# ZSHCRWY25/3DRVO-MARL-CollisionAvoidance

Measured on AMD Instinct MI355X. Metric: drone-steps/sec (env.step throughput), higher is better.
Workload: dtype f64; 1 GPU; BASELINE config 3 env.step: 64 drones x 4096 envs per GPU, nm=10, 0 buildings, map [50.0, 50.0, 10.0], fused step+auto-reset, f32 actions in HBM; envs_per_gpu=4096, drones=64, diag_build=False, cold_all=False, ablate=0, device_error_word=0

## Files before the change

### 3drvo-marl-collisionavoidance_amd/csrc/rvo3d_aux_kernels.hpp

```cpp
#pragma once

#include "rvo3d_step.hpp"

namespace rvo3d {

__global__ void reset_kernel(const Params P, const uint8_t* env_mask, const uint8_t* drone_mask) {
  const int g = blockIdx.x * blockDim.x + threadIdx.x;
  if (g >= P.E * P.N) return;
  if (env_mask && !env_mask[g / P.N]) return;
  if (drone_mask && !drone_mask[g]) return;
  double s[3];
  load_wp(P, g, 0, s);
  P.px()[g] = s[0]; P.py()[g] = s[1]; P.pz()[g] = s[2];
  P.vx()[g] = 0.0; P.vy()[g] = 0.0; P.vz()[g] = 0.0;
  P.wp_idx()[g] = 1; P.arrive()[g] = 0; P.dest()[g] = 0;
  P.real_len()[g] = 0.0; P.max_dev()[g] = 0.0; P.yaw()[g] = 0.0; P.pitch()[g] = 0.0;
  double c1[3];
  load_wp(P, g, 1, c1);
  RVO3D_STORE_CUR(P, g, c1);
  RVO3D_STORE_PREV(P, g, s);
  const bool plain = P.dev0()[g] == 0.0;
  P.dvk_a()[g] = plain ? P.dv0_a()[g] : kDvInvalid;
  P.dvk_b()[g] = P.dv0_b()[g];
}

__global__ void wpcache_kernel(const Params P) {
  const int g = blockIdx.x * blockDim.x + threadIdx.x;
  if (g >= P.E * P.N) return;
  const int np = P.n_points()[g];
  int i = P.wp_idx()[g];
  i = i < 1 ? 1 : (i > np - 1 ? np - 1 : i);
  double v[3];
  load_wp(P, g, i, v);
  RVO3D_STORE_CUR(P, g, v);
  load_wp(P, g, i - 1, v);
  RVO3D_STORE_PREV(P, g, v);
}

__global__ void dv0_kernel(const Params P) {
  const int g = blockIdx.x * blockDim.x + threadIdx.x;
  if (g >= P.E * P.N) return;
  double p[3], cur[3], dv[3];
  load_wp(P, g, 0, p);
  load_wp(P, g, 1, cur);
  des_vel(P, p, cur, dv);
  uint32_t a, b;
  dv_encode(dv, a, b);
  P.dv0_a()[g] = a; P.dv0_b()[g] = b;
  P.dev0()[g] = deviation(p, cur, p);
}

__global__ void des_vel_kernel(const Params P, double* out) {
  const int g = blockIdx.x * blockDim.x + threadIdx.x;
  if (g >= P.E * P.N) return;
  double p[3] = {P.px()[g], P.py()[g], P.pz()[g]}, cur[3], dv[3];
  RVO3D_LOAD_CUR(P, g, cur);
  des_vel(P, p, cur, dv);
  out[3 * (size_t)g] = dv[0]; out[3 * (size_t)g + 1] = dv[1]; out[3 * (size_t)g + 2] = dv[2];
}

struct RvoVelArgs { double vmax[3]; double acceler; };

__device__ __forceinline__ int arange_len(double lo, double hi) {
  const double n = __builtin_ceil((hi - lo) / 0.5);
  return n > 0 ? (int)n : 0;
}
__device__ __forceinline__ double arange_at(double lo, int k) {
  const double next = lo + 0.5;
  return k == 0 ? lo : (k == 1 ? next : lo + k * (next - lo));
}

__global__ void __launch_bounds__(512) rvo_vel_kernel(const Params P, const RvoVelArgs A, double* out) {
  extern __shared__ __attribute__((aligned(16))) unsigned char smem[];
  const int N = P.N, d = threadIdx.x, e = blockIdx.x;
  const int T = blockDim.x;
  double* const lx = reinterpret_cast<double*>(smem);
  const bool active = d < N;
  const int g = active ? e * N + d : e * N;
  Drone S;
  S.x = P.px()[g]; S.y = P.py()[g]; S.z = P.pz()[g];
  S.vx = P.vx()[g]; S.vy = P.vy()[g]; S.vz = P.vz()[g];
// ... 130 lines not shown
```

### 3drvo-marl-collisionavoidance_amd/csrc/rvo3d_capi.hip

```cpp
#include "../../include/rvo3d.h"
#include "rvo3d_device.hpp"

#include <atomic>
#include <cmath>
#include <cstdio>
#include <cstdlib>
#include <cstring>
#include <exception>
#include <new>
#include <string>
#include <vector>

using rvo3d::Params;

namespace {
thread_local std::string g_err;

int fail(int code, const std::string& msg) {
  g_err = msg;
  return code;
}
#define HIP_TRY(expr)                                                            \
  do {                                                                           \
    hipError_t _e = (expr);                                                      \
// ... 317 lines not shown
  *out = nullptr;
  if (cfg->num_envs < 1 || cfg->num_drones < 1 || cfg->num_drones > rvo3d::kMaxThreads)
    return fail(RVO3D_ERR_INVALID, "need num_envs >= 1 and 1 <= num_drones <= 512");
  if (cfg->max_points < 2 || cfg->num_buildings < 0 || cfg->neighbors_num < 0)
    return fail(RVO3D_ERR_INVALID, "need max_points >= 2, num_buildings >= 0, neighbors_num >= 0");
  if ((long long)cfg->num_envs * cfg->num_drones > (1ll << 30))
    return fail(RVO3D_ERR_INVALID, "num_envs * num_drones too large");
  if (cfg->action_decimals > 9) return fail(RVO3D_ERR_INVALID, "action_decimals must be <= 9");
  DeviceGuard dg;
  if (int rc0 = dg.enter(cfg->device)) return rc0;

  rvo3d_env* h = new (std::nothrow) rvo3d_env();
  if (!h) return fail(RVO3D_ERR_INVALID, "out of host memory");
  struct Owner {
    rvo3d_env* p;
    ~Owner() {
      if (!p) return;
      if (p->arena) (void)hipFree(p->arena);
      delete p;
    }
  } owner{h};
  h->cfg = *cfg;
  Params& P = h->P;
  rvo3d::Cold& C = h->cold;
  std::memset(&P, 0, sizeof P);
  std::memset(&C, 0, sizeof C);
  P.E = cfg->num_envs; P.N = cfg->num_drones; P.P = cfg->max_points;
  C.nb = cfg->num_buildings; P.nm = cfg->neighbors_num; P.env_train = cfg->env_train ? 1 : 0;
  P.W = 12 + 9 * P.nm;
#ifdef RVO3D_DIAG
  if (const char* ab = std::getenv("RVO3D_ABLATE")) P.ablate = std::atoi(ab);
#endif
  C.act_scale = cfg->action_decimals >= 0 ? std::pow(10.0, cfg->action_decimals) : 0.0;
  for (int k = 0; k < 3; ++k) C.map[k] = cfg->map_size[k];
  P.T10 = sq_threshold(10.0);
  C.T5 = sq_threshold(5.0);
  C.bgx = C.bgy = 0; C.bg_inv = 0.0;
  if (cfg->num_buildings > 0 && cfg->map_size[0] > 0 && cfg->map_size[1] > 0 &&
      std::isfinite(cfg->map_size[0]) && std::isfinite(cfg->map_size[1])) {
    const double cs = std::fmax(8.0, std::fmax(cfg->map_size[0], cfg->map_size[1]) / 64.0);
    C.bgx = (int)std::ceil(cfg->map_size[0] / cs); C.bgy = (int)std::ceil(cfg->map_size[1] / cs);
    if (C.bgx < 1) C.bgx = 1;
    if (C.bgy < 1) C.bgy = 1;
    C.bg_inv = 1.0 / cs;
  }
  C.T04 = sq_threshold(0.4);
  {
    double mx = std::fmax(C.map[0], std::fmax(C.map[1], C.map[2]));
    if (!(mx > 0)) mx = 1.0;
    for (int k = 0; k < 3; ++k) C.cen[k] = 0.5 * C.map[k];
    const double cmax = 0.75 * mx + 16.0;
    const double u = std::ldexp(1.0, -24);
    const double eD = u * (2.0 * cmax + 21.0);
    const double band = 2.0 * (2.0 * 1.7320508 * 10.5 * eD + 3.0 * eD * eD + 8.0 * u * 110.25);
    C.cmax = (float)cmax;
    P.band = std::nextafter((float)band, INFINITY);
    const float t10f = std::nextafter((float)(P.T10 + band), INFINITY);
    P.t10n = -std::nextafter(t10f, INFINITY);
    P.bandn = P.band + P.t10n;
    C.kdot = std::nextafter((float)(2.0 * (eD + 4.0 * u * 10.5) * 1.001), INFINITY);
    const double gap = 512.0 * band;
    const double cs = 4.0 * (1.7320508 * eD / std::sqrt(gap) + 8.0 * u);
    P.x1_gap = (float)gap;
    P.x1_k2 = (float)(1.0 - (4e-3 + 4.0 * cs));
    const double cs_out = cs > 1e-3 ? cs : 1e-3;
    P.x1_cs2 = (float)(cs_out * cs_out);
// ... 85 lines not shown
  RVO3D_API_BEGIN
  DeviceGuard dg;
  int rc = check(h, false, dg);
  if (rc) return rc;
  if (!waypoints || !n_points) return fail(RVO3D_ERR_INVALID, "waypoints / n_points are required");
  const Params& P = h->P;
  const rvo3d::Cold& C = h->cold;
  if (C.nb > 0 && !buildings) return fail(RVO3D_ERR_INVALID, "buildings required when num_buildings > 0");
  hipStream_t s = static_cast<hipStream_t>(stream);
  const size_t EN = (size_t)P.E * P.N;
  std::vector<double> wp((size_t)P.P * 3 * EN), rl(EN), rad(EN), pri(EN), p95(P.P);
  for (size_t g = 0; g < EN; ++g) {
    const int np = n_points[g];
    if (np < 2 || np > P.P) return fail(RVO3D_ERR_INVALID, "n_points entries must be in [2, max_points]");
    const double* src = waypoints + g * P.P * 3;
    double total = 0.0;
    for (int k = 0; k < P.P; ++k) {
      const int kk = k < np ? k : np - 1;
      for (int c = 0; c < 3; ++c) wp[((size_t)k * 3 + c) * EN + g] = src[kk * 3 + c];
      if (k + 1 < np) {
        const double dx = src[(k + 1) * 3] - src[k * 3], dy = src[(k + 1) * 3 + 1] - src[k * 3 + 1],
                     dz = src[(k + 1) * 3 + 2] - src[k * 3 + 2];
        total += std::sqrt(py_sq(dx) + py_sq(dy) + py_sq(dz));
      }
    }
    rl[g] = total;
    rad[g] = radius ? radius[g] : 0.2;
    pri[g] = priority ? priority[g] : 5.0;
  }
  {
    bool uni = true;
    for (size_t g = 1; g < EN && uni; ++g)
      uni = std::memcmp(&rad[g], &rad[0], 8) == 0 && std::memcmp(&pri[g], &pri[0], 8) == 0;
    h->P.uniform_rp = uni ? 1 : 0;
    h->P.r0 = rad[0];
    h->P.prio0 = pri[0];
  }
  for (int k = 0; k < P.P; ++k) p95[k] = std::pow(0.95, (double)k);
  HIP_TRY(hipMemcpy2DAsync((void*)P.wp(0, 0), (size_t)P.S * 8, wp.data(), EN * 8, EN * 8,
                           (size_t)P.P * 3, hipMemcpyHostToDevice, s));
  HIP_TRY(hipMemcpyAsync((void*)P.n_points(), n_points, EN * 4, hipMemcpyHostToDevice, s));
  HIP_TRY(hipMemcpyAsync((void*)P.route_len(), rl.data(), EN * 8, hipMemcpyHostToDevice, s));
  HIP_TRY(hipMemcpyAsync((void*)P.radius(), rad.data(), EN * 8, hipMemcpyHostToDevice, s));
  HIP_TRY(hipMemcpyAsync((void*)P.prio(), pri.data(), EN * 8, hipMemcpyHostToDevice, s));
  HIP_TRY(hipMemcpyAsync((void*)C.pow95, p95.data(), (size_t)P.P * 8, hipMemcpyHostToDevice, s));
  std::vector<uint16_t> grid;
  if (C.nb > 0) {
    HIP_TRY(hipMemcpyAsync((void*)C.bld, buildings, (size_t)C.nb * 32, hipMemcpyHostToDevice, s));
    if (C.bgx > 0) {
      const int K = rvo3d::kBgridK;
      const double cs = 1.0 / C.bg_inv;
      double rmax = 0.0;
      for (size_t g = 0; g < EN; ++g) {
        if (rad[g] != rad[g]) rmax = INFINITY;
        else if (rad[g] > rmax) rmax = rad[g];
      }
      grid.assign((size_t)C.bgx * C.bgy * (K + 1), 0);
      for (int ix = 0; ix < C.bgx; ++ix)
        for (int iy = 0; iy < C.bgy; ++iy) {
          uint16_t* cell = &grid[((size_t)ix * C.bgy + iy) * (K + 1)];
          const double x0 = ix == 0 ? -INFINITY : ix * cs, x1 = ix == C.bgx - 1 ? INFINITY : (ix + 1) * cs;
          const double y0 = iy == 0 ? -INFINITY : iy * cs, y1 = iy == C.bgy - 1 ? INFINITY : (iy + 1) * cs;
          int n = 0;
          bool overflow = false;
          for (int b = 0; b < C.nb && !overflow; ++b) {
            const double bx = buildings[4 * b], by = buildings[4 * b + 1];
            double reach = rmax + buildings[4 * b + 3];
            if (!(reach < 5.0)) reach = 5.0;
            reach += 1e-3;
// ... 552 lines not shown
```

### 3drvo-marl-collisionavoidance_amd/csrc/rvo3d_math.hpp

```cpp
#pragma once

#include "rvo3d_params.hpp"

namespace rvo3d {

__device__ __forceinline__ double sq(double x) { return x * x; }
__device__ __forceinline__ double dot3b(double ax, double ay, double az, double bx,
                                        double by, double bz) {
  return __builtin_fma(az, bz, __builtin_fma(ay, by, ax * bx));
}
__device__ __forceinline__ double norm3b(double x, double y, double z) {
  return __builtin_sqrt(dot3b(x, y, z, x, y, z));
}
__device__ __forceinline__ double norm2sq(double x, double y) { return __builtin_fma(y, y, x * x); }
__device__ __forceinline__ bool finite_d(double q) { return __builtin_fabs(q) < __builtin_inf(); }

__device__ __forceinline__ float round2_f32(double x) {
  const double k = __builtin_rint(x * 100.0);
  return __builtin_fabs(k) < 16777216.0 ? (float)(k * 0.01) : (float)(k / 100.0);
}
__device__ __forceinline__ double k_over_1000(double k) {
  const double q = k * 0.001;
  const double r = __builtin_fma(-q, 1000.0, k);
  const double c = q + r * 0.001;
  return finite_d(k) ? c : k;
}

constexpr uint32_t kDvInvalid = 0xffffffffu;
__device__ __forceinline__ void dv_encode(const double dv[3], uint32_t& a, uint32_t& b) {
  const double k0 = __builtin_rint(dv[0] * 1000.0), k1 = __builtin_rint(dv[1] * 1000.0),
               k2 = __builtin_rint(dv[2] * 1000.0);
  const bool ok = __builtin_fabs(k0) <= 1023.0 && __builtin_fabs(k1) <= 1023.0 &&
                  __builtin_fabs(k2) <= 1023.0 && k_over_1000(k0) == dv[0] &&
                  k_over_1000(k1) == dv[1] && k_over_1000(k2) == dv[2];
  const uint32_t nz = (uint32_t)(k0 == 0.0 && __builtin_signbit(dv[0])) |
                      ((uint32_t)(k1 == 0.0 && __builtin_signbit(dv[1])) << 1) |
                      ((uint32_t)(k2 == 0.0 && __builtin_signbit(dv[2])) << 2);
  a = ok ? ((uint32_t)((int)k0 + 1024) | ((uint32_t)((int)k1 + 1024) << 16)) : kDvInvalid;
  b = (uint32_t)((int)(ok ? k2 : 0.0) + 1024) | (nz << 16);
}
__device__ __forceinline__ bool dv_decode(uint32_t a, uint32_t b, double dv[3]) {
  if (a == kDvInvalid) return false;
  const int k0 = (int)(a & 0xffffu) - 1024, k1 = (int)(a >> 16) - 1024, k2 = (int)(b & 0xffffu) - 1024;
  dv[0] = (b & (1u << 16)) ? -0.0 : k_over_1000((double)k0);
  dv[1] = (b & (1u << 17)) ? -0.0 : k_over_1000((double)k1);
  dv[2] = (b & (1u << 18)) ? -0.0 : k_over_1000((double)k2);
  return true;
}

__device__ __forceinline__ double py_round2_c(double x) {
  double p = x * 100.0;
  double e = __builtin_fma(x, 100.0, -p);
  double c = __builtin_floor(p);
  double d = (p - (c + 0.5)) + e;
  if (d > 0.0) c += 1.0;
  else if (d == 0.0 && (((long long)c) & 1)) c += 1.0;
  return c;
}
__device__ __forceinline__ double clampd(double x, double lo, double hi) {
  return x < lo ? lo : (x > hi ? hi : x);
}
__device__ __forceinline__ double np_mod(double a, double b) {
  double m;
  if (b > 0.0 && a > -b && a < 2.0 * b) m = a >= b ? a - b : a;
  else m = fmod(a, b);
  if (m != 0.0) {
    if ((b < 0.0) != (m < 0.0)) m += b;
  } else {
    m = __builtin_copysign(0.0, b);
  }
  return m;
}

__device__ __forceinline__ void des_vel(const Params& P, const double p[3], const double cur[3],
                                        double out[3]) {
  const double dx = cur[0] - p[0], dy = cur[1] - p[1], dz = cur[2] - p[2];
  const double d2 = dot3b(dx, dy, dz, dx, dy, dz);
  if (d2 > P.cold().T04) {
    const double inv = 1000.0 / __builtin_sqrt(d2);
    const double ux = dx * inv, uy = dy * inv, uz = dz * inv;
    double kx = __builtin_rint(ux), ky = __builtin_rint(uy), kz = __builtin_rint(uz);
    const double m = __builtin_fmin(__builtin_fmin(0.5 - __builtin_fabs(ux - kx),
                                                   0.5 - __builtin_fabs(uy - ky)),
                                    0.5 - __builtin_fabs(uz - kz));
    if (!(m > 1e-7)) {
      const double az = atan2(dy, dx);
      const double el = atan2(dz, __builtin_sqrt(norm2sq(dx, dy)));
      double sa, ca, se, ce;
      sincos(az, &sa, &ca);
      sincos(el, &se, &ce);
      kx = __builtin_rint((1.0 * (ca * ce)) * 1000.0);
      ky = __builtin_rint((1.0 * (sa * ce)) * 1000.0);
      kz = __builtin_rint((1.0 * se) * 1000.0);
    }
    out[0] = k_over_1000(kx); out[1] = k_over_1000(ky); out[2] = k_over_1000(kz);
  } else {
    out[0] = out[1] = out[2] = 0.0;
  }
}

__device__ __forceinline__ double deviation(const double a[3], const double b[3],
                                            const double p[3]) {
  double dx = b[0] - a[0], dy = b[1] - a[1], dz = b[2] - a[2];
  double mag = __builtin_sqrt(sq(dx) + sq(dy) + sq(dz));
  if (mag == 0.0) return 0.0;
  double hx = dx / mag, hy = dy / mag, hz = dz / mag;
  double qx0 = p[0] - a[0], qy0 = p[1] - a[1], qz0 = p[2] - a[2];
  double t = qx0 * hx + qy0 * hy + qz0 * hz;
  double qx = a[0] + t * hx, qy = a[1] + t * hy, qz = a[2] + t * hz;
  return __builtin_sqrt(sq(p[0] - qx) + sq(p[1] - qy) + sq(p[2] - qz));
}

__device__ __forceinline__ bool arrived(const Params& P, const double p[3], const double d[3]) {
  const double x = p[0] - d[0], y = p[1] - d[1], z = p[2] - d[2];
  return dot3b(x, y, z, x, y, z) <= P.cold().T04;
}

__device__ __forceinline__ double vo_exp_time(double rx, double ry, double rz, double rvx,
                                              double rvy, double rvz, double ra, double rb) {
  double r = ra + rb;
  double ux = -rvx, uy = -rvy, uz = -rvz;
  double a = sq(ux) + sq(uy) + sq(uz);
  double b = 2 * rx * ux + 2 * ry * uy + 2 * rz * uz;
  double c = sq(rx) + sq(ry) + sq(rz) - sq(r);
  if (c <= 0) return 0.0;
  double temp = sq(b) - 4 * a * c;
  if (temp <= 0) return __builtin_inf();
  double s = __builtin_sqrt(temp);
  double t1 = (-b + s) / (2 * a);
  double t2 = (-b - s) / (2 * a);
  if (t1 < 0 && t2 < 0) return -1.0;
// ... 17 lines not shown
```

### 3drvo-marl-collisionavoidance_amd/csrc/rvo3d_params.hpp

```cpp
#pragma once

#include <hip/hip_runtime.h>
#include <stdint.h>

namespace rvo3d {

constexpr double kExpRadius = 0.2;
constexpr double kCtimeThreshold = 2.0;
constexpr double kDeg2Rad = 0.017453292519943295;
constexpr double kPi = 3.141592653589793;
constexpr int kMaxThreads = 512;
constexpr double kCosD = 0.999999995;
constexpr double kSinD = 1.0000000000e-4;

struct Cold {
  double map[3];
  double T5, T04;
  double cen[3];
  double act_scale;
  float cmax;
  float kdot;
  uint32_t zf_div;
  uint32_t zf_magic;
  uint32_t zf_q;
  int zf_iters;
  uint32_t zmask[128];
  int nb;
  const double* bld;
  const double* pow95;
  const uint16_t* bgrid;
  int bgx, bgy;
  double bg_inv;
};
constexpr int kBgridK = 15;
typedef const __attribute__((address_space(4))) Cold ColdC;

struct Params {
  int E, N, P, nm, env_train, epb, W;
  int action_f64;
  int dv_cached;
  int g_cached;
  int action_mode;
  float acceler;
#ifdef RVO3D_DIAG
  int ablate;
#endif
  int zf16;
  int uniform_rp;
  double r0, prio0;
  double T10;
  float t10n;
  float bandn;
  float band;
  int nw;
  float x1_gap;
  float x1_k2;
  float x1_cs2;
  double* f64;
  int32_t* i32;
  uint8_t* u8;
  uint32_t S;
  enum { F_PX, F_PY, F_PZ, F_VX, F_VY, F_VZ, F_YAW, F_PITCH, F_REAL_LEN, F_MAX_DEV, F_EXTRA_LEN,
         F_CUR, F_PREV = F_CUR + 3,
         F_ROUTE_LEN = F_PREV + 3, F_RADIUS, F_PRIO, F_DEV0, F_WP };
  __host__ __device__ double* f(int k) const { return f64 + (size_t)k * S; }
  __host__ __device__ double* px() const { return f(F_PX); }
  __host__ __device__ double* py() const { return f(F_PY); }
  __host__ __device__ double* pz() const { return f(F_PZ); }
  __host__ __device__ double* vx() const { return f(F_VX); }
  __host__ __device__ double* vy() const { return f(F_VY); }
  __host__ __device__ double* vz() const { return f(F_VZ); }
  __host__ __device__ double* yaw() const { return f(F_YAW); }
  __host__ __device__ double* pitch() const { return f(F_PITCH); }
  __host__ __device__ double* real_len() const { return f(F_REAL_LEN); }
  __host__ __device__ double* max_dev() const { return f(F_MAX_DEV); }
  __host__ __device__ double* extra_len() const { return f(F_EXTRA_LEN); }
  __host__ __device__ int32_t* wp_idx() const { return i32; }
  __host__ __device__ uint8_t* arrive() const { return u8; }
  __host__ __device__ uint8_t* dest() const { return u8 + S; }
  __host__ __device__ double* route_len() const { return f(F_ROUTE_LEN); }
  __host__ __device__ double* radius() const { return f(F_RADIUS); }
  __host__ __device__ double* prio() const { return f(F_PRIO); }
// ... 44 lines not shown
```

### 3drvo-marl-collisionavoidance_amd/csrc/rvo3d_step.hpp

```cpp
#pragma once

#include "rvo3d_pairs.hpp"

namespace rvo3d {

__device__ __forceinline__ bool building_test(const double* const bld, int b, const Drone& S,
                                              double T5) {
  const double bx = bld[4 * b], by = bld[4 * b + 1], bh = bld[4 * b + 2], br = bld[4 * b + 3];
  const double ex = S.x - bx, ey = S.y - by;
  if ((bh > S.z - 2) & (norm2sq(ex, ey) <= T5) & (S.z <= bh))
    return __builtin_sqrt(sq(ex) + sq(ey)) <= S.r + br;
  return false;
}
__device__ __forceinline__ bool building_hit(const Params& P, const Drone& S) {
  const int nb = P.cold().nb;
  if (nb == 0) return false;
  bool hit = false;
  const double* const bld = P.cold().bld;
  const double T5 = P.cold().T5;
  const int gx = P.cold().bgx;
  if (gx > 0) {
    const int gy = P.cold().bgy;
    const double inv = P.cold().bg_inv;
    int ix = (int)__builtin_floor(S.x * inv), iy = (int)__builtin_floor(S.y * inv);
    ix = ix < 0 ? 0 : (ix > gx - 1 ? gx - 1 : ix);
    iy = iy < 0 ? 0 : (iy > gy - 1 ? gy - 1 : iy);
    const uint16_t* const cell = P.cold().bgrid + (size_t)(ix * gy + iy) * (kBgridK + 1);
    const uint4 c0 = *reinterpret_cast<const uint4*>(cell);
    const int cnt = (int)(c0.x & 0xffffu);
    if (cnt != 0xffff) {
      if (cnt >= 1) {
        const int b0 = (int)(c0.x >> 16), b1 = cnt >= 2 ? (int)(c0.y & 0xffffu) : b0;
        hit |= building_test(bld, b0, S, T5);
        hit |= building_test(bld, b1, S, T5);
      }
      if (cnt >= 3) {
        const int b0 = (int)(c0.y >> 16), b1 = cnt >= 4 ? (int)(c0.z & 0xffffu) : b0;
        hit |= building_test(bld, b0, S, T5);
        hit |= building_test(bld, b1, S, T5);
      }
      for (int k = 5; k <= cnt; ++k) hit |= building_test(bld, (int)cell[k], S, T5);
      return hit;
    }
  }
#pragma unroll 4
  for (int b = 0; b < nb; ++b) hit |= building_test(bld, b, S, T5);
  return hit;
}

struct ProprioTail { float dv0, dv1, dv2, dev; bool bad; };
__device__ __forceinline__ ProprioTail proprio_tail(const double dv[3], double dev) {
  ProprioTail t;
  t.dv0 = round2_f32(dv[0]); t.dv1 = round2_f32(dv[1]); t.dv2 = round2_f32(dv[2]);
  t.dev = round2_f32(dev);
  t.bad = !(finite_d(dv[0]) && finite_d(dv[1]) && finite_d(dv[2]) && finite_d(dev));
  asm volatile("" : "+v"(t.dv0), "+v"(t.dv1), "+v"(t.dv2), "+v"(t.dev));
  return t;
}
__device__ __forceinline__ void write_proprio(const Params& P, int g, const Drone& S,
                                              const ProprioTail& t) {
  float* o = P.obs + (size_t)g * P.W;
  const double v[8] = {S.x, S.y, S.z, S.vx, S.vy, S.vz, S.r, S.prio};
  float f[12];
  bool bad = t.bad;
#pragma unroll
  for (int k = 0; k < 8; ++k) {
    f[k] = round2_f32(v[k]);
    bad |= !finite_d(v[k]);
  }
  f[8] = t.dv0; f[9] = t.dv1; f[10] = t.dv2; f[11] = t.dev;
  if ((P.W & 1) == 0) {
    float2* o2 = reinterpret_cast<float2*>(o);
#pragma unroll
    for (int k = 0; k < 6; ++k) o2[k] = make_float2(f[2 * k], f[2 * k + 1]);
  } else {
#pragma unroll
    for (int k = 0; k < 12; ++k) o[k] = f[k];
  }
  if (bad) atomicOr(P.err, 1u);
}

__device__ __forceinline__ void stage_row(const Params& P, const Lds& L, int tid, int g,
                                          const Drone& S, const ProprioTail& t, int kept) {
  const double v[8] = {S.x, S.y, S.z, S.vx, S.vy, S.vz, S.r, S.prio};
  float f[12];
  bool bad = t.bad;
#pragma unroll
  for (int k = 0; k < 8; ++k) {
    f[k] = round2_f32(v[k]);
    bad |= !finite_d(v[k]);
  }
  f[8] = t.dv0; f[9] = t.dv1; f[10] = t.dv2; f[11] = t.dev;
  float4* pro = reinterpret_cast<float4*>(L.w[0]) + 3 * tid;
  pro[0] = make_float4(f[0], f[1], f[2], f[3]);
  pro[1] = make_float4(f[4], f[5], f[6], f[7]);
  pro[2] = make_float4(f[8], f[9], f[10], f[11]);
  L.kept[tid] = ((12 + 9 * kept + 1) & ~1) >> 1;
  if (((9 * kept) & 1) && kept < P.nm) P.obs[(size_t)g * P.W + 12 + 9 * kept] = 0.0f;
  if (bad) atomicOr(P.err, 1u);
}

template <int NW>
__device__ __forceinline__ void row_fill_pairs(const Params& P, const Lds& L, int tid, int row0,
                                               int nrows) {
  const int q = P.W >> 1;
  const int ln = tid & 63, wv = tid >> 6;
  const int nwv = NW == 1 ? 1 : (L.T >> 6);
  const int pair0 = row0 >> 1;
  const int npairs = ((row0 + nrows + 1) >> 1) - pair0;
  const int rbase = 2 * pair0 - row0;
  const float2* pro2 = reinterpret_cast<const float2*>(L.w[0]);
  const uint32_t pair_bytes = 8u * (uint32_t)P.W;
  char* const obsb = reinterpret_cast<char*>(P.obs) + (size_t)pair0 * pair_bytes;
  for (int cb = 0; cb < q; cb += 64) {
    const int c = cb + ln;
    const bool lane_on = c < q;
    const int h0 = 2 * c, h1 = 2 * c + 1;
    const int s0 = h0 >= q ? 1 : 0, s1 = h1 >= q ? 1 : 0;
    const int u0 = h0 - (s0 ? q : 0), u1 = h1 - (s1 ? q : 0);
    const bool p0 = u0 < 6, p1 = u1 < 6;
    const int pu0 = p0 ? u0 : 5, pu1 = p1 ? u1 : 5;
    uint32_t off = (uint32_t)wv * pair_bytes + 16u * (uint32_t)c;
    const uint32_t ostep = (uint32_t)nwv * pair_bytes;
    for (int i0 = wv; i0 < npairs; i0 += 4 * nwv) {
// ... 88 lines not shown
  const bool proa = uia < 6u, prob = uib < 6u;
  const int pia = (int)(proa ? uia : 5u), pib = (int)(prob ? uib : 5u);
  const int da_row = pa ? 1 : 0, db_row = pb ? 1 : 0;
  char* pc = base + (rs0 & ~63u) + 16u * (uint32_t)ch;
  const size_t step = (size_t)8 * (size_t)nwv * rb;
  for (int r = r0; r < nrows; r += 8 * nwv, pc += step) {
    const int ra = r - da_row, rbw = r - db_row;
    const int za = L.kept[ra], zb = L.kept[rbw];
    const float2 da = pro2[ra * 6 + pia], db = pro2[rbw * 6 + pib];
    const bool va = proa | (uia >= (uint32_t)za), vb = prob | (uib >= (uint32_t)zb);
    const float2 a = proa ? da : make_float2(0.f, 0.f), b = prob ? db : make_float2(0.f, 0.f);
    if (va & vb) *reinterpret_cast<float4*>(pc) = make_float4(a.x, a.y, b.x, b.y);
    if (va != vb) *reinterpret_cast<float2*>(pc + (vb ? 8 : 0)) = vb ? b : a;
  }
}

__device__ __forceinline__ void write_vo_rows(const Params& P, const Lds& L, int tid, int lbase,
                                              int g, const Drone& S, int kept) {
  float* o = P.obs + (size_t)g * P.W;
  bool bad = false;
  for (int s = 0; s < kept; ++s) {
    const uint32_t pk = P.row_pk(s)[g];
    const int j = (int)(pk & 0xffffu);
    const Drone O = lds_drone(L, lbase + j);
    const double pr = (S.prio == O.prio) ? 0.5 : S.prio / (S.prio + O.prio);
    double row[9];
    row[0] = pr * (2 * S.x + (S.vx + O.vx));
    row[1] = pr * (2 * S.y + (S.vy + O.vy));
    row[2] = pr * (2 * S.z + (S.vz + O.vz));
    row[3] = O.x - S.x; row[4] = O.y - S.y; row[5] = O.z - S.z;
    row[6] = (double)(pk >> 16) / 100.0;
    row[7] = pair_md(S, O);
    row[8] = P.row_iet(s)[g];
#pragma unroll
    for (int k = 0; k < 9; ++k) {
      bad |= !finite_d(row[k]);
      o[12 + 9 * s + k] = round2_f32(row[k]);
    }
  }
  P.vo_count[g] = kept;
  if (bad) atomicOr(P.err, 1u);
}

__device__ __forceinline__ void publish_zero_run(const Params& P, int g, int kept) {
  if ((P.W & 1) == 0 && ((9 * kept) & 1) && kept < P.nm) P.obs[(size_t)g * P.W + 12 + 9 * kept] = 0.0f;
}

__device__ __forceinline__ void zero_fill(const Params& P, const Lds& L, int tid, int row0,
                                          int nrows) {
  const uint32_t per_row = P.cold().zf_div;
  if (per_row == 0) return;
  const uint32_t total = (uint32_t)nrows * per_row;
  float* base = P.obs + (size_t)row0 * P.W + 12;
  if ((P.W & 1) == 0) {
    for (uint32_t q = tid; q < total; q += L.T) {
      const uint32_t row = (uint32_t)(((uint64_t)q * P.cold().zf_magic) >> 32);
      const uint32_t c = q - row * per_row;
      const uint32_t first = (9u * (uint32_t)L.kept[row] + 1u) >> 1;
      if (c >= first)
        *reinterpret_cast<float2*>(base + (size_t)row * P.W + 2 * c) = make_float2(0.f, 0.f);
    }
  } else {
    for (uint32_t q = tid; q < total; q += L.T) {
      const uint32_t row = (uint32_t)(((uint64_t)q * P.cold().zf_magic) >> 32);
      const uint32_t c = q - row * per_row;
      if (c >= 9u * (uint32_t)L.kept[row]) base[(size_t)row * P.W + c] = 0.0f;
    }
  }
}

__device__ __forceinline__ void load_wp(const Params& P, int g, int k, double out[3]) {
// ... 102 lines not shown
  const int full_rows = P.epb * (PAD ? Nr : N);
  const int nrows = ((P.E - e0) < P.epb ? (P.E - e0) : P.epb) * (PAD ? Nr : N);
  const int row0 = e0 * (PAD ? Nr : N);
  const int lrow = PAD ? el * Nr + d : tid;
  constexpr bool LITE = (MODE == kStepAutoReset);
  constexpr bool GSH = NW > 1 && NFIX == 64 * NW;
  constexpr bool XQ = NW == 1 && NFIX != 0;

  RVO3D_STAMP(0);
#if RVO3D_DEPHASE
  if (NW == 1) {
    unsigned hw_slot;
    asm volatile("s_getreg_b32 %0, hwreg(HW_REG_HW_ID)" : "=s"(hw_slot));
    if (hw_slot & 1)
      for (int i = 0; i < RVO3D_DEPHASE; ++i) __builtin_amdgcn_s_sleep(32);
  }
#endif
  Drone S;
  S.x = S.y = S.z = S.vx = S.vy = S.vz = 0.0; S.r = 0.2; S.prio = 5;
  if (PAD && d >= Nr) {
    S.x = S.y = S.z = __builtin_inf();
    const int o = el * 2 * N + d, os = el * N + d;
#pragma unroll
    for (int k = 0; k < 12; ++k) {
      const float v = (k == WX || k == WY || k == WZ) ? 1e30f : (k == WKD ? -1.0f : 0.0f);
      if (k == WX || k == WY || k == WZ || k == WR) {
        L.w[k][o] = v;
        if (d <= (N >> 1)) L.w[k][o + N] = v;
      } else L.w[k][os] = v;
    }
  }
  double a[3] = {0, 0, 0}, cur[3] = {0, 0, 0}, dv[3] = {0, 0, 0};
  double dev = 0, max_dev = 0;
  int wpi = 1;

  uint32_t gw[NW];
  const bool have_gw = MODE != kObserve && P.g_cached != 0;
  uint32_t old_cnt = 0;
  if (active) {
    if (LITE && NW == 1 && P.prev_cnt) {
      old_cnt = (uint32_t)P.prev_cnt[g];
      old_cnt = old_cnt < (uint32_t)P.nm ? old_cnt : (uint32_t)P.nm;
    }
    S.x = P.px()[g]; S.y = P.py()[g]; S.z = P.pz()[g];
    S.vx = P.vx()[g]; S.vy = P.vy()[g]; S.vz = P.vz()[g];
    if (P.uniform_rp) { S.r = P.r0; S.prio = P.prio0; }
    else { S.r = P.radius()[g]; S.prio = P.prio()[g]; }
    if (have_gw) {
#pragma unroll
      for (int w = 0; w < NW; ++w) gw[w] = P.gcache(w)[g];
    }
    if (MODE != kObserve) {
      if (P.action_mode == 1) {
        const float* A = static_cast<const float*>(P.actions) + (size_t)g * 3;
        const double vv[3] = {S.vx, S.vy, S.vz};
#pragma unroll
        for (int k = 0; k < 3; ++k) {
          const float r = __builtin_rintf(A[k] * 100.0f) / 100.0f;
          const double x = (double)(P.acceler * r) + vv[k];
          a[k] = __builtin_rint(x * 100.0) / 100.0;
        }
      } else {
        if (P.action_f64) {
          const double* A = static_cast<const double*>(P.actions) + (size_t)g * 3;
          a[0] = A[0]; a[1] = A[1]; a[2] = A[2];
        } else {
          const float* A = static_cast<const float*>(P.actions) + (size_t)g * 3;
          a[0] = (double)A[0]; a[1] = (double)A[1]; a[2] = (double)A[2];
        }
        if (P.cold().act_scale > 0) {
          a[0] = __builtin_rint(a[0] * P.cold().act_scale) / P.cold().act_scale;
          a[1] = __builtin_rint(a[1] * P.cold().act_scale) / P.cold().act_scale;
          a[2] = __builtin_rint(a[2] * P.cold().act_scale) / P.cold().act_scale;
        }
      }
    }
  }
  RVO3D_STAMP(1);
  double az[3] = {a[0], a[1], a[2]};
  if (norm3b(a[0], a[1], a[2]) < 1e-5) az[0] = az[1] = az[2] = 0.0;
  const double zero3[3] = {0, 0, 0};

  if (tid < P.epb) { L.any_reset[tid] = 0; L.far[tid] = 0; }
  if (LITE && NW > 1 && tid == 0) *L.any_old = 0;
  L.kept[tid] = 0;
  __syncthreads();
  if (LITE && NW == 1 && active && P.prev_cnt) L.kept[lrow] = (int)old_cnt;
  L.x[tid] = S.x; L.y[tid] = S.y; L.z[tid] = S.z;
  L.vx[tid] = S.vx; L.vy[tid] = S.vy; L.vz[tid] = S.vz;
  L.r[tid] = S.r; L.prio[tid] = S.prio;
  {
    const double p[3] = {S.x, S.y, S.z}, v[3] = {S.vx, S.vy, S.vz};
    stage_f32<NW>(P, L, el, d, active, p, v, az, S.r, S.prio);
  }
  __syncthreads();

  bool flag, collision = false;
  double tmin;

  if (MODE == kObserve) {
    if (active) {
      double prev[3];
      max_dev = P.max_dev()[g];
      RVO3D_LOAD_CUR(P, g, cur);
      RVO3D_LOAD_PREV(P, g, prev);
      const double p[3] = {S.x, S.y, S.z};
      des_vel(P, p, cur, dv);
      dev = deviation(prev, cur, p);
      if (dev > max_dev) max_dev = dev;
    }
    const int kept = sweep_env<NW, true, true, TRAIN, GSH, XQ>(P, L, tid, el, d, g, active, S, zero3, true, true, flag,
                                               tmin, collision, gw, false);
    if (active) {
      write_vo_rows(P, L, tid, lbase, g, S, kept);
      if (P.zf16) stage_row(P, L, lrow, g, S, proprio_tail(dv, dev), kept);
      else {
        write_proprio(P, g, S, proprio_tail(dv, dev));
        publish_zero_run(P, g, kept);
        L.kept[lrow] = kept;
      }
      P.max_dev()[g] = max_dev;
      uint32_t dvk_a, dvk_b;
      dv_encode(dv, dvk_a, dvk_b);
      P.dvk_a()[g] = dvk_a; P.dvk_b()[g] = dvk_b;
#pragma unroll
      for (int w = 0; w < NW; ++w) P.gcache(w)[g] = gw[w];
    }
    __syncthreads();
    if (P.zf16) row_fill_pairs<NW>(P, L, tid, row0, nrows);
    else zero_fill(P, L, tid, row0, nrows);
    return;
  }

  RVO3D_STAMP(2);
  sweep_env<NW, false, false, TRAIN, GSH, XQ>(P, L, tid, el, d, g, active && !RVO3D_ABLATED(1), S, az, false, false, flag,
                              tmin, collision, gw, have_gw);
  double rew_k = 0;
  double mov_nc = 0;
  bool f_dest = false;
  RVO3D_STAMP(3);
  constexpr bool kLoadAhead = NW <= 2;
  double prev[3] = {0, 0, 0}, yaw = 0, pitch = 0, real_len = 0, route_len = 0;
  int npts = 2;
  bool f_arrive_in = false, f_dest_in = false;
#define RVO3D_LOAD_INTEGRATION_STATE()                                               \
  {                                                                                  \
    wpi = P.wp_idx()[g];                                                             \
    RVO3D_LOAD_PREV(P, g, prev);                                                     \
    yaw = P.yaw()[g]; pitch = P.pitch()[g]; real_len = P.real_len()[g];              \
    route_len = P.route_len()[g];                                                    \
    npts = P.n_points()[g];                                                          \
    f_arrive_in = P.arrive()[g] != 0; f_dest_in = P.dest()[g] != 0;                  \
  }
  if (active) {
    max_dev = P.max_dev()[g];
    RVO3D_LOAD_CUR(P, g, cur);
    uint32_t dvk_a = 0, dvk_b = 0;
    if (P.dv_cached) { dvk_a = P.dvk_a()[g]; dvk_b = P.dvk_b()[g]; }
    if (kLoadAhead) RVO3D_LOAD_INTEGRATION_STATE()
    bool have = false;
    if (P.dv_cached) have = dv_decode(dvk_a, dvk_b, dv);
    if (!have) {
      if (!kLoadAhead) RVO3D_LOAD_PREV(P, g, prev);
      const double p[3] = {S.x, S.y, S.z};
      des_vel(P, p, cur, dv);
      dev = deviation(prev, cur, p);
      if (dev > max_dev) max_dev = dev;
    }
    rew_k = rvo_reward_k(rvo_reward_pre(dv, a), flag, tmin);
  }
  RVO3D_STAMP(18);
  __syncthreads();
  if (active) {
    if (!kLoadAhead) RVO3D_LOAD_INTEGRATION_STATE()
#undef RVO3D_LOAD_INTEGRATION_STATE
    bool ex_set = false;
    double extra_len = 0.0;
    const int wpi_in = wpi;
    bool f_arrive = f_arrive_in;
    f_dest = f_dest_in;

    double speed = norm3b(S.vx, S.vy, S.vz);
    const double acc = clampd(a[0] * 1.0, -1.0, 1.0);
    const double dyaw = clampd(a[1] * 90.0, -90.0, 90.0);
    const double dpit = clampd(a[2] * 90.0, -90.0, 90.0);
    const double nv = speed + acc;
    speed = (0.0 > nv) ? 0.0 : nv;
    yaw = np_mod(yaw + dyaw, 360.0);
    pitch = clampd(pitch + dpit, -90.0, 90.0);
    double nvx = 0.0, nvy = 0.0, nvz = 0.0;
    if (!f_dest) {
      double sy, cy, sp, cp;
      sincos(yaw * kDeg2Rad, &sy, &cy);
      sincos(pitch * kDeg2Rad, &sp, &cp);
      nvx = speed * cp * cy; nvy = speed * cp * sy; nvz = speed * sp;
    }
    const double q0 = S.x, q1 = S.y, q2 = S.z;
    S.x = S.x + nvx; S.y = S.y + nvy; S.z = S.z + nvz;
    S.vx = nvx; S.vy = nvy; S.vz = nvz;
    real_len = real_len + norm3b(S.x - q0, S.y - q1, S.z - q2);
    const double p[3] = {S.x, S.y, S.z};
    double dst[3] = {0, 0, 0};
    if (f_arrive || arrived(P, p, cur)) load_wp(P, g, npts - 1, dst);
    if (arrived(P, p, cur)) {
      const bool at_dst = arrived(P, p, dst);
      if (at_dst) { extra_len = real_len - route_len; ex_set = true; }
      if (!at_dst && wpi < npts - 1) {
        wpi += 1;
        prev[0] = cur[0]; prev[1] = cur[1]; prev[2] = cur[2];
        load_wp(P, g, wpi, cur);
        RVO3D_STORE_CUR(P, g, cur);
        RVO3D_STORE_PREV(P, g, prev);
        f_arrive = false;
      }
    }
    des_vel(P, p, cur, dv);
    dev = deviation(prev, cur, p);
    if (dev > max_dev) max_dev = dev;
    bool arrive_r = false, dest_r = false;
    const int waypoint_num = wpi;
    if (!f_arrive && arrived(P, p, cur)) { f_arrive = true; arrive_r = true; }
    if (f_arrive) {
      if (arrived(P, p, dst)) {
        extra_len = real_len - route_len;
        ex_set = true;
        if (!f_dest) { f_dest = true; dest_r = true; }
      }
    }
    const double exlen = real_len - route_len + 4;
    mov_nc = mov_reward_k(P, false, arrive_r, waypoint_num, npts - 1, dest_r, dev, exlen > 0,
                          exlen);
    RVO3D_STAMP(19);
    collision = building_hit(P, S);
    if (S.x < 0 || S.x > P.cold().map[0] || S.y < 0 || S.y > P.cold().map[1] || S.z < 0 || S.z > P.cold().map[2])
      collision = true;
    P.yaw()[g] = yaw; P.pitch()[g] = pitch; P.real_len()[g] = real_len;
    if (ex_set) P.extra_len()[g] = extra_len;
    if (wpi != wpi_in) P.wp_idx()[g] = wpi;
    if (f_arrive != f_arrive_in) P.arrive()[g] = f_arrive ? 1 : 0;
    if (f_dest != f_dest_in) P.dest()[g] = f_dest ? 1 : 0;
    P.info[g] = f_arrive ? 1 : 0;
    P.finish[g] = f_dest ? 1 : 0;
  }
  L.x[tid] = S.x; L.y[tid] = S.y; L.z[tid] = S.z;
  L.vx[tid] = S.vx; L.vy[tid] = S.vy; L.vz[tid] = S.vz;
  {
    const double p[3] = {S.x, S.y, S.z}, v[3] = {S.vx, S.vy, S.vz};
    stage_f32<NW>(P, L, el, d, active, p, v, az, S.r, S.prio);
  }
  __syncthreads();

  RVO3D_STAMP(4);
  int kept = 0;
  if (LITE) {
    if (collide_env<NW, TRAIN, GSH>(P, L, tid, el, d, active && !RVO3D_ABLATED(2), S, gw)) collision = true;
  } else {
    kept = sweep_env<NW, true, true, TRAIN, GSH, XQ>(P, L, tid, el, d, g, active && !RVO3D_ABLATED(2), S, az, false,
                                     false, flag, tmin, collision, gw, false);
  }
  bool do_reset = false;
  if (active) {
    const double rew64 = k_over_1000(rew_k) + k_over_1000(collision ? -50000.0 : mov_nc);
    P.reward[g] = (float)rew64;
    if (P.reward64) P.reward64[g] = rew64;
    P.done[g] = collision ? 1 : 0;
    do_reset = LITE && (collision || f_dest);
  }

  RVO3D_STAMP(5);
  if (LITE) {
    if (active && P.reset_mask) P.reset_mask[g] = do_reset ? 1 : 0;
    if (do_reset) L.any_reset[el] = 1;
    __syncthreads();
    double p[3] = {0, 0, 0}, rcur[3] = {0, 0, 0}, rdev = 0.0;
    uint32_t rdv_a = 0, rdv_b = 0;
    if (NW > 1 && active && P.prev_cnt) {
      old_cnt = (uint32_t)P.prev_cnt[g];
      old_cnt = old_cnt < (uint32_t)P.nm ? old_cnt : (uint32_t)P.nm;
      L.kept[lrow] = (int)old_cnt;
      if (old_cnt != 0) *L.any_old = 1;
    }
    if (do_reset) {
      load_wp(P, g, 0, p);
      rdev = P.dev0()[g];
      load_wp(P, g, 1, rcur);
      rdv_a = P.dv0_a()[g]; rdv_b = P.dv0_b()[g];
    }
    RVO3D_STAMP(26);
    if (NW == 1 && two_phase_rows(P, row0, nrows, full_rows) && !RVO3D_ABLATED(16)) early_zero_blocks<NW>(P, L, tid, row0, nrows);
    RVO3D_STAMP(27);
    if (do_reset) {
      S.x = p[0]; S.y = p[1]; S.z = p[2]; S.vx = S.vy = S.vz = 0.0;
      dev = rdev;
      cur[0] = rcur[0]; cur[1] = rcur[1]; cur[2] = rcur[2];
      if (!dv_decode(rdv_a, rdv_b, dv)) {
        des_vel(P, p, cur, dv);
        dev = deviation(p, cur, p);
      }
      RVO3D_STORE_CUR(P, g, cur);
      RVO3D_STORE_PREV(P, g, p);
      max_dev = dev > 0.0 ? dev : 0.0;
      P.wp_idx()[g] = 1; P.arrive()[g] = 0; P.dest()[g] = 0;
      P.real_len()[g] = 0.0; P.yaw()[g] = 0.0; P.pitch()[g] = 0.0;
      L.x[tid] = S.x; L.y[tid] = S.y; L.z[tid] = S.z;
      L.vx[tid] = 0.0; L.vy[tid] = 0.0; L.vz[tid] = 0.0;
      const double v0[3] = {0, 0, 0};
      stage_f32<NW>(P, L, el, d, true, p, v0, az, S.r, S.prio);
    }
    if (active && L.any_reset[el] != 0) {
      const int os = el * N + d;
      L.w[WAX][os] = 0.f; L.w[WAY][os] = 0.f; L.w[WAZ][os] = 0.f;
    }
  }
  if (active) {
    uint32_t dvk_a, dvk_b;
    dv_encode(dv, dvk_a, dvk_b);
    P.dvk_a()[g] = dvk_a; P.dvk_b()[g] = dvk_b;
  }
  const ProprioTail ptail = proprio_tail(dv, dev);
  if (active) P.max_dev()[g] = max_dev;
  if (LITE) {
    __syncthreads();
    RVO3D_STAMP(6);
    const bool env_reset = (active || (PAD && el < P.epb)) && (L.any_reset[el] != 0);
    bool c2 = false;
    const double aa[3] = {env_reset ? 0.0 : az[0], env_reset ? 0.0 : az[1], env_reset ? 0.0 : az[2]};
    bool have_gw2 = !env_reset;
    if (NW == 1) {
      const unsigned long long rlanes = __ballot(do_reset);
      if (L.far[el] != 0) {
        uint32_t valid[1];
        valid_offsets<1>(N, d, valid);
        gw[0] = valid[0];
      } else {
        gw[0] = regate_resets(P, L, tid, el, d, active, rlanes, gw[0]);
      }
      have_gw2 = true;
    }
    if (RVO3D_ABLATED(2)) have_gw2 = false;
    if (NW > 1 && two_phase_rows(P, row0, nrows, full_rows) && !RVO3D_ABLATED(16)) early_zero_blocks<NW>(P, L, tid, row0, nrows);
    kept = sweep_env<NW, true, false, TRAIN, GSH, XQ>(P, L, tid, el, d, g, active && !RVO3D_ABLATED(4), S, aa,
                                      false, env_reset, flag, tmin, c2, gw, have_gw2);
  }
  RVO3D_STAMP(7);
  const bool two_phase = LITE && two_phase_rows(P, row0, nrows, full_rows);
  if (NW > 1 && two_phase) {
    asm volatile("s_waitcnt vmcnt(0)" ::: "memory");
    __syncthreads();
  }
  if (active) {
    if (!RVO3D_ABLATED(8)) {
      if (two_phase) asm volatile("s_waitcnt vmcnt(0)" ::: "memory");
// ... 26 lines not shown
```

Baseline: 7.755 billion drone-steps/s.

## Carry packed desired-velocity code through step and batch round-to-2 observations

The packed desired-velocity key is now produced directly inside des_vel and dv_decode, so dv_encode no longer re-derives the rounded integers and checks them each step. Observation rounding is grouped: a wave-wide ballot checks that all values are small, and if so takes a fast multiply path that skips the per-value range and finiteness checks. Radius and priority floats are precomputed on the host when uniform. Action rounding replaces divisions with a reciprocal plus FMA correction. This cuts f64 divide and branch work in the step kernel, but adds more code paths whose bit-exactness depends on the new correction and threshold logic.

```diff
diff --git a/3drvo-marl-collisionavoidance_amd/csrc/rvo3d_aux_kernels.hpp b/3drvo-marl-collisionavoidance_amd/csrc/rvo3d_aux_kernels.hpp
--- a/3drvo-marl-collisionavoidance_amd/csrc/rvo3d_aux_kernels.hpp
+++ b/3drvo-marl-collisionavoidance_amd/csrc/rvo3d_aux_kernels.hpp
@@ -43,10 +43,9 @@
   double p[3], cur[3], dv[3];
   load_wp(P, g, 0, p);
   load_wp(P, g, 1, cur);
-  des_vel(P, p, cur, dv);
-  uint32_t a, b;
-  dv_encode(dv, a, b);
-  P.dv0_a()[g] = a; P.dv0_b()[g] = b;
+  DvK K;
+  des_vel(P, p, cur, dv, K);
+  P.dv0_a()[g] = K.a; P.dv0_b()[g] = K.b;
   P.dev0()[g] = deviation(p, cur, p);
 }
 
diff --git a/3drvo-marl-collisionavoidance_amd/csrc/rvo3d_capi.hip b/3drvo-marl-collisionavoidance_amd/csrc/rvo3d_capi.hip
--- a/3drvo-marl-collisionavoidance_amd/csrc/rvo3d_capi.hip
+++ b/3drvo-marl-collisionavoidance_amd/csrc/rvo3d_capi.hip
@@ -373,6 +373,7 @@
   if (const char* ab = std::getenv("RVO3D_ABLATE")) P.ablate = std::atoi(ab);
 #endif
   C.act_scale = cfg->action_decimals >= 0 ? std::pow(10.0, cfg->action_decimals) : 0.0;
+  C.act_inv = C.act_scale > 0 ? 1.0 / C.act_scale : 0.0;
   for (int k = 0; k < 3; ++k) C.map[k] = cfg->map_size[k];
   P.T10 = sq_threshold(10.0);
   C.T5 = sq_threshold(5.0);
@@ -524,9 +525,12 @@
     bool uni = true;
     for (size_t g = 1; g < EN && uni; ++g)
       uni = std::memcmp(&rad[g], &rad[0], 8) == 0 && std::memcmp(&pri[g], &pri[0], 8) == 0;
+    uni = uni && std::fabs(rad[0]) < rvo3d::kRound2Small && std::fabs(pri[0]) < rvo3d::kRound2Small;
     h->P.uniform_rp = uni ? 1 : 0;
     h->P.r0 = rad[0];
     h->P.prio0 = pri[0];
+    h->P.r0f = (float)(std::nearbyint(rad[0] * 100.0) / 100.0);
+    h->P.prio0f = (float)(std::nearbyint(pri[0] * 100.0) / 100.0);
   }
   for (int k = 0; k < P.P; ++k) p95[k] = std::pow(0.95, (double)k);
   HIP_TRY(hipMemcpy2DAsync((void*)P.wp(0, 0), (size_t)P.S * 8, wp.data(), EN * 8, EN * 8,
diff --git a/3drvo-marl-collisionavoidance_amd/csrc/rvo3d_math.hpp b/3drvo-marl-collisionavoidance_amd/csrc/rvo3d_math.hpp
--- a/3drvo-marl-collisionavoidance_amd/csrc/rvo3d_math.hpp
+++ b/3drvo-marl-collisionavoidance_amd/csrc/rvo3d_math.hpp
@@ -19,32 +19,58 @@
   const double k = __builtin_rint(x * 100.0);
   return __builtin_fabs(k) < 16777216.0 ? (float)(k * 0.01) : (float)(k / 100.0);
 }
-__device__ __forceinline__ double k_over_1000(double k) {
+constexpr double kRound2Small = 167772.0;
+template <int NV>
+__device__ __forceinline__ bool round2_group(const double (&v)[NV], float (&f)[NV]) {
+  bool small = true;
+#pragma unroll
+  for (int k = 0; k < NV; ++k) small &= __builtin_fabs(v[k]) < kRound2Small;
+  bool bad = false;
+  if (__builtin_expect(__builtin_amdgcn_ballot_w64(!small) == 0, 1)) {
+#pragma unroll
+    for (int k = 0; k < NV; ++k) f[k] = (float)(__builtin_rint(v[k] * 100.0) * 0.01);
+  } else {
+#pragma unroll
+    for (int k = 0; k < NV; ++k) {
+      f[k] = round2_f32(v[k]);
+      bad |= !finite_d(v[k]);
+    }
+  }
+  return bad;
+}
+__device__ __forceinline__ double k_over_1000_finite(double k) {
   const double q = k * 0.001;
   const double r = __builtin_fma(-q, 1000.0, k);
-  const double c = q + r * 0.001;
+  return q + r * 0.001;
+}
+__device__ __forceinline__ double k_over_1000(double k) {
+  const double c = k_over_1000_finite(k);
   return finite_d(k) ? c : k;
+}
+__device__ __forceinline__ double k_over_pow10(double k, double s, double inv) {
+  const double q = k * inv;
+  const double r = __builtin_fma(-q, s, k);
+  const double c = q + r * inv;
+  return __builtin_amdgcn_class(k, 0x198) ? c : k;
 }
 
 constexpr uint32_t kDvInvalid = 0xffffffffu;
-__device__ __forceinline__ void dv_encode(const double dv[3], uint32_t& a, uint32_t& b) {
-  const double k0 = __builtin_rint(dv[0] * 1000.0), k1 = __builtin_rint(dv[1] * 1000.0),
-               k2 = __builtin_rint(dv[2] * 1000.0);
-  const bool ok = __builtin_fabs(k0) <= 1023.0 && __builtin_fabs(k1) <= 1023.0 &&
-                  __builtin_fabs(k2) <= 1023.0 && k_over_1000(k0) == dv[0] &&
-                  k_over_1000(k1) == dv[1] && k_over_1000(k2) == dv[2];
-  const uint32_t nz = (uint32_t)(k0 == 0.0 && __builtin_signbit(dv[0])) |
-                      ((uint32_t)(k1 == 0.0 && __builtin_signbit(dv[1])) << 1) |
-                      ((uint32_t)(k2 == 0.0 && __builtin_signbit(dv[2])) << 2);
-  a = ok ? ((uint32_t)((int)k0 + 1024) | ((uint32_t)((int)k1 + 1024) << 16)) : kDvInvalid;
-  b = (uint32_t)((int)(ok ? k2 : 0.0) + 1024) | (nz << 16);
+struct DvK { uint32_t a, b; };
+__device__ __forceinline__ DvK dv_pack(int k0, int k1, int k2, uint32_t nz, bool ok) {
+  DvK K;
+  K.a = ok ? ((uint32_t)(k0 + 1024) | ((uint32_t)(k1 + 1024) << 16)) : kDvInvalid;
+  K.b = (uint32_t)((ok ? k2 : 0) + 1024) | (nz << 16);
+  return K;
 }
-__device__ __forceinline__ bool dv_decode(uint32_t a, uint32_t b, double dv[3]) {
+__device__ __forceinline__ bool dv_decode(uint32_t a, uint32_t b, double dv[3], DvK& K) {
+  const uint32_t f0 = a & 0xffffu, f1 = a >> 16, f2 = b & 0xffffu;
+  const bool z0 = (b & (1u << 16)) != 0, z1 = (b & (1u << 17)) != 0, z2 = (b & (1u << 18)) != 0;
+  K = dv_pack(z0 ? 0 : (int)f0 - 1024, z1 ? 0 : (int)f1 - 1024, z2 ? 0 : (int)f2 - 1024, (b >> 16) & 7u,
+              (z0 || f0 - 1u < 2047u) && (z1 || f1 - 1u < 2047u) && (z2 || f2 - 1u < 2047u));
   if (a == kDvInvalid) return false;
-  const int k0 = (int)(a & 0xffffu) - 1024, k1 = (int)(a >> 16) - 1024, k2 = (int)(b & 0xffffu) - 1024;
-  dv[0] = (b & (1u << 16)) ? -0.0 : k_over_1000((double)k0);
-  dv[1] = (b & (1u << 17)) ? -0.0 : k_over_1000((double)k1);
-  dv[2] = (b & (1u << 18)) ? -0.0 : k_over_1000((double)k2);
+  dv[0] = z0 ? -0.0 : k_over_1000_finite((double)((int)f0 - 1024));
+  dv[1] = z1 ? -0.0 : k_over_1000_finite((double)((int)f1 - 1024));
+  dv[2] = z2 ? -0.0 : k_over_1000_finite((double)((int)f2 - 1024));
   return true;
 }
 
@@ -73,7 +99,7 @@
 }
 
 __device__ __forceinline__ void des_vel(const Params& P, const double p[3], const double cur[3],
-                                        double out[3]) {
+                                        double out[3], DvK& K) {
   const double dx = cur[0] - p[0], dy = cur[1] - p[1], dz = cur[2] - p[2];
   const double d2 = dot3b(dx, dy, dz, dx, dy, dz);
   if (d2 > P.cold().T04) {
@@ -83,7 +109,7 @@
     const double m = __builtin_fmin(__builtin_fmin(0.5 - __builtin_fabs(ux - kx),
                                                    0.5 - __builtin_fabs(uy - ky)),
                                     0.5 - __builtin_fabs(uz - kz));
-    if (!(m > 1e-7)) {
+    if (!(m > 1e-7) || !finite_d(d2)) {
       const double az = atan2(dy, dx);
       const double el = atan2(dz, __builtin_sqrt(norm2sq(dx, dy)));
       double sa, ca, se, ce;
@@ -94,9 +120,17 @@
       kz = __builtin_rint((1.0 * se) * 1000.0);
     }
     out[0] = k_over_1000(kx); out[1] = k_over_1000(ky); out[2] = k_over_1000(kz);
+    K = dv_pack((int)kx, (int)ky, (int)kz, 0u,
+                __builtin_fabs(kx) <= 1023.0 && __builtin_fabs(ky) <= 1023.0 && __builtin_fabs(kz) <= 1023.0);
   } else {
     out[0] = out[1] = out[2] = 0.0;
+    K = dv_pack(0, 0, 0, 0u, true);
   }
+}
+__device__ __forceinline__ void des_vel(const Params& P, const double p[3], const double cur[3],
+                                        double out[3]) {
+  DvK K;
+  des_vel(P, p, cur, out, K);
 }
 
 __device__ __forceinline__ double deviation(const double a[3], const double b[3],
diff --git a/3drvo-marl-collisionavoidance_amd/csrc/rvo3d_params.hpp b/3drvo-marl-collisionavoidance_amd/csrc/rvo3d_params.hpp
--- a/3drvo-marl-collisionavoidance_amd/csrc/rvo3d_params.hpp
+++ b/3drvo-marl-collisionavoidance_amd/csrc/rvo3d_params.hpp
@@ -18,6 +18,7 @@
   double T5, T04;
   double cen[3];
   double act_scale;
+  double act_inv;
   float cmax;
   float kdot;
   uint32_t zf_div;
@@ -48,6 +49,7 @@
   int zf16;
   int uniform_rp;
   double r0, prio0;
+  float r0f, prio0f;
   double T10;
   float t10n;
   float bandn;
diff --git a/3drvo-marl-collisionavoidance_amd/csrc/rvo3d_step.hpp b/3drvo-marl-collisionavoidance_amd/csrc/rvo3d_step.hpp
--- a/3drvo-marl-collisionavoidance_amd/csrc/rvo3d_step.hpp
+++ b/3drvo-marl-collisionavoidance_amd/csrc/rvo3d_step.hpp
@@ -49,25 +49,45 @@
 }
 
 struct ProprioTail { float dv0, dv1, dv2, dev; bool bad; };
+template <bool GROUPED = true>
 __device__ __forceinline__ ProprioTail proprio_tail(const double dv[3], double dev) {
   ProprioTail t;
-  t.dv0 = round2_f32(dv[0]); t.dv1 = round2_f32(dv[1]); t.dv2 = round2_f32(dv[2]);
-  t.dev = round2_f32(dev);
-  t.bad = !(finite_d(dv[0]) && finite_d(dv[1]) && finite_d(dv[2]) && finite_d(dev));
+  if (GROUPED) {
+    const double v[4] = {dv[0], dv[1], dv[2], dev};
+    float f[4];
+    t.bad = round2_group(v, f);
+    t.dv0 = f[0]; t.dv1 = f[1]; t.dv2 = f[2]; t.dev = f[3];
+  } else {
+    t.dv0 = round2_f32(dv[0]); t.dv1 = round2_f32(dv[1]); t.dv2 = round2_f32(dv[2]);
+    t.dev = round2_f32(dev);
+    t.bad = !(finite_d(dv[0]) && finite_d(dv[1]) && finite_d(dv[2]) && finite_d(dev));
+  }
   asm volatile("" : "+v"(t.dv0), "+v"(t.dv1), "+v"(t.dv2), "+v"(t.dev));
   return t;
+}
+__device__ __forceinline__ bool proprio_head(const Params& P, const Drone& S, float (&f)[12]) {
+  bool bad;
+  if (P.uniform_rp) {
+    const double v[6] = {S.x, S.y, S.z, S.vx, S.vy, S.vz};
+    float h[6];
+    bad = round2_group(v, h);
+#pragma unroll
+    for (int k = 0; k < 6; ++k) f[k] = h[k];
+    f[6] = P.r0f; f[7] = P.prio0f;
+  } else {
+    const double v[8] = {S.x, S.y, S.z, S.vx, S.vy, S.vz, S.r, S.prio};
+    float h[8];
+    bad = round2_group(v, h);
+#pragma unroll
+    for (int k = 0; k < 8; ++k) f[k] = h[k];
+  }
+  return bad;
 }
 __device__ __forceinline__ void write_proprio(const Params& P, int g, const Drone& S,
                                               const ProprioTail& t) {
   float* o = P.obs + (size_t)g * P.W;
-  const double v[8] = {S.x, S.y, S.z, S.vx, S.vy, S.vz, S.r, S.prio};
   float f[12];
-  bool bad = t.bad;
-#pragma unroll
-  for (int k = 0; k < 8; ++k) {
-    f[k] = round2_f32(v[k]);
-    bad |= !finite_d(v[k]);
-  }
+  const bool bad = proprio_head(P, S, f) | t.bad;
   f[8] = t.dv0; f[9] = t.dv1; f[10] = t.dv2; f[11] = t.dev;
   if ((P.W & 1) == 0) {
     float2* o2 = reinterpret_cast<float2*>(o);
@@ -82,14 +102,8 @@
 
 __device__ __forceinline__ void stage_row(const Params& P, const Lds& L, int tid, int g,
                                           const Drone& S, const ProprioTail& t, int kept) {
-  const double v[8] = {S.x, S.y, S.z, S.vx, S.vy, S.vz, S.r, S.prio};
   float f[12];
-  bool bad = t.bad;
-#pragma unroll
-  for (int k = 0; k < 8; ++k) {
-    f[k] = round2_f32(v[k]);
-    bad |= !finite_d(v[k]);
-  }
+  const bool bad = proprio_head(P, S, f) | t.bad;
   f[8] = t.dv0; f[9] = t.dv1; f[10] = t.dv2; f[11] = t.dev;
   float4* pro = reinterpret_cast<float4*>(L.w[0]) + 3 * tid;
   pro[0] = make_float4(f[0], f[1], f[2], f[3]);
@@ -244,11 +258,10 @@
     row[6] = (double)(pk >> 16) / 100.0;
     row[7] = pair_md(S, O);
     row[8] = P.row_iet(s)[g];
-#pragma unroll
-    for (int k = 0; k < 9; ++k) {
-      bad |= !finite_d(row[k]);
-      o[12 + 9 * s + k] = round2_f32(row[k]);
-    }
+    float f[9];
+    bad |= round2_group(row, f);
+#pragma unroll
+    for (int k = 0; k < 9; ++k) o[12 + 9 * s + k] = f[k];
   }
   P.vo_count[g] = kept;
   if (bad) atomicOr(P.err, 1u);
@@ -417,6 +430,7 @@
   }
   double a[3] = {0, 0, 0}, cur[3] = {0, 0, 0}, dv[3] = {0, 0, 0};
   double dev = 0, max_dev = 0;
+  DvK dvk = {0u, 0u};
   int wpi = 1;
 
   uint32_t gw[NW];
@@ -443,7 +457,7 @@
         for (int k = 0; k < 3; ++k) {
           const float r = __builtin_rintf(A[k] * 100.0f) / 100.0f;
           const double x = (double)(P.acceler * r) + vv[k];
-          a[k] = __builtin_rint(x * 100.0) / 100.0;
+          a[k] = k_over_pow10(__builtin_rint(x * 100.0), 100.0, 0.01);
         }
       } else {
         if (P.action_f64) {
@@ -453,10 +467,12 @@
           const float* A = static_cast<const float*>(P.actions) + (size_t)g * 3;
           a[0] = (double)A[0]; a[1] = (double)A[1]; a[2] = (double)A[2];
         }
-        if (P.cold().act_scale > 0) {
-          a[0] = __builtin_rint(a[0] * P.cold().act_scale) / P.cold().act_scale;
-          a[1] = __builtin_rint(a[1] * P.cold().act_scale) / P.cold().act_scale;
-          a[2] = __builtin_rint(a[2] * P.cold().act_scale) / P.cold().act_scale;
+        const double sc = P.cold().act_scale;
+        if (sc > 0) {
+          const double inv = P.cold().act_inv;
+          a[0] = k_over_pow10(__builtin_rint(a[0] * sc), sc, inv);
+          a[1] = k_over_pow10(__builtin_rint(a[1] * sc), sc, inv);
+          a[2] = k_over_pow10(__builtin_rint(a[2] * sc), sc, inv);
         }
       }
     }
@@ -490,7 +506,7 @@
       RVO3D_LOAD_CUR(P, g, cur);
       RVO3D_LOAD_PREV(P, g, prev);
       const double p[3] = {S.x, S.y, S.z};
-      des_vel(P, p, cur, dv);
+      des_vel(P, p, cur, dv, dvk);
       dev = deviation(prev, cur, p);
       if (dev > max_dev) max_dev = dev;
     }
@@ -505,9 +521,7 @@
         L.kept[lrow] = kept;
       }
       P.max_dev()[g] = max_dev;
-      uint32_t dvk_a, dvk_b;
-      dv_encode(dv, dvk_a, dvk_b);
-      P.dvk_a()[g] = dvk_a; P.dvk_b()[g] = dvk_b;
+      P.dvk_a()[g] = dvk.a; P.dvk_b()[g] = dvk.b;
 #pragma unroll
       for (int w = 0; w < NW; ++w) P.gcache(w)[g] = gw[w];
     }
@@ -544,7 +558,7 @@
     if (P.dv_cached) { dvk_a = P.dvk_a()[g]; dvk_b = P.dvk_b()[g]; }
     if (kLoadAhead) RVO3D_LOAD_INTEGRATION_STATE()
     bool have = false;
-    if (P.dv_cached) have = dv_decode(dvk_a, dvk_b, dv);
+    if (P.dv_cached) have = dv_decode(dvk_a, dvk_b, dv, dvk);
     if (!have) {
       if (!kLoadAhead) RVO3D_LOAD_PREV(P, g, prev);
       const double p[3] = {S.x, S.y, S.z};
@@ -599,7 +613,7 @@
         f_arrive = false;
       }
     }
-    des_vel(P, p, cur, dv);
+    des_vel(P, p, cur, dv, dvk);
     dev = deviation(prev, cur, p);
     if (dev > max_dev) max_dev = dev;
     bool arrive_r = false, dest_r = false;
@@ -637,6 +651,8 @@
 
   RVO3D_STAMP(4);
   int kept = 0;
+  ProprioTail ptail;
+  if (!LITE) ptail = proprio_tail(dv, dev);
   if (LITE) {
     if (collide_env<NW, TRAIN, GSH>(P, L, tid, el, d, active && !RVO3D_ABLATED(2), S, gw)) collision = true;
   } else {
@@ -678,8 +694,8 @@
       S.x = p[0]; S.y = p[1]; S.z = p[2]; S.vx = S.vy = S.vz = 0.0;
       dev = rdev;
       cur[0] = rcur[0]; cur[1] = rcur[1]; cur[2] = rcur[2];
-      if (!dv_decode(rdv_a, rdv_b, dv)) {
-        des_vel(P, p, cur, dv);
+      if (!dv_decode(rdv_a, rdv_b, dv, dvk)) {
+        des_vel(P, p, cur, dv, dvk);
         dev = deviation(p, cur, p);
       }
       RVO3D_STORE_CUR(P, g, cur);
@@ -698,11 +714,9 @@
     }
   }
   if (active) {
-    uint32_t dvk_a, dvk_b;
-    dv_encode(dv, dvk_a, dvk_b);
-    P.dvk_a()[g] = dvk_a; P.dvk_b()[g] = dvk_b;
-  }
-  const ProprioTail ptail = proprio_tail(dv, dev);
+    P.dvk_a()[g] = dvk.a; P.dvk_b()[g] = dvk.b;
+  }
+  if (LITE) ptail = proprio_tail<!(NW == 4 && !TRAIN)>(dv, dev);
   if (active) P.max_dev()[g] = max_dev;
   if (LITE) {
     __syncthreads();
```

Result: no change. 7.789 billion drone-steps/s, median of 5 (+0.4%).
